# franioli/icepy4d

Hardware: AMD Instinct MI355X
Metric: matched stereo image-pairs/sec (4096 kpts, 1080p) (higher is better)
Workload: dtype f32

## Files before the change

### icepy4d_amd/csrc/attention_bx.hip

```cpp
#include "bf16x3.h"
#include "common.h"
#include "kernels.h"
#include "sp_post.h"

#include <cstdlib>

namespace im {

static constexpr int BKT = 32;
static constexpr int BKS = 144;
static constexpr int BVS = 192;
static constexpr int BK_PLANE = BKT * BKS, BV_PLANE = BKT * BVS;
static constexpr int B_STAGE = 3 * BK_PLANE + 3 * BV_PLANE;
static constexpr int B_LDS = 2 * B_STAGE;
static constexpr int DPL = BKT * 128;
static constexpr int D_LDS = 3 * 3 * (DPL + DPL);

__device__ __forceinline__ f32x16 mfma_attn(u32x4 a, u32x4 b, f32x16 c) {
#ifdef BX_ABL_NO_MFMA
    c[0] += __uint_as_float(a.x ^ b.x);
    return c;
#else
    return mfma_bf(a, b, c);
#endif
}

__device__ __forceinline__ void stage4(unsigned char* plane0, int plane_bytes, int off, float4 x) {
    unsigned h0, m0, l0, h1, m1, l1;
    split2(x.x, x.y, h0, m0, l0);
    split2(x.z, x.w, h1, m1, l1);
    *reinterpret_cast<u32x2*>(plane0 + off) = u32x2{h0, h1};
    *reinterpret_cast<u32x2*>(plane0 + plane_bytes + off) = u32x2{m0, m1};
    *reinterpret_cast<u32x2*>(plane0 + 2 * plane_bytes + off) = u32x2{l0, l1};
}

typedef __attribute__((address_space(3))) bf16x4 lds_bf16x4;
__device__ __forceinline__ u32x2 tr_read(const unsigned char* p) {
#ifdef BX_ABL_NO_VREAD
    const unsigned x = (unsigned)(unsigned long long)p;
    return u32x2{x, 0x3f803f80u};
#else
    const bf16x4 v = __builtin_amdgcn_ds_read_tr16_b64_v4bf16((lds_bf16x4*)(p));
    return __builtin_bit_cast(u32x2, v);
#endif
}
__device__ __forceinline__ u32x4 kf_read(const unsigned char* p) {
#ifdef BX_ABL_NO_KREAD
    const unsigned x = (unsigned)(unsigned long long)p;
    return u32x4{x, 0x3f803f80u, x, 0x3f803f80u};
#else
    return *reinterpret_cast<const u32x4*>(p);
#endif
}

static constexpr float BX_SLACK = 8.f;
__device__ __forceinline__ float bmax3(float a, float b, float c) { return __builtin_fmaxf(__builtin_fmaxf(a, b), c); }

template <bool TAIL>
__device__ __forceinline__ float softmax_ref(f32x16& s, int kb, int nk, int hh, float& m_run, float& l_run, f32x16& o0, f32x16& o1) {
    if (TAIL) {
#pragma unroll
        for (int r = 0; r < 16; ++r)
            if (kb + acc_row(r, hh) >= nk) s[r] = -INFINITY;
    }
    float mx0 = bmax3(s[0], s[1], s[2]), mx1 = bmax3(s[3], s[4], s[5]);
    mx0 = bmax3(mx0, s[6], s[7]); mx1 = bmax3(mx1, s[8], s[9]);
    mx0 = bmax3(mx0, s[10], s[11]); mx1 = bmax3(mx1, s[12], s[13]);
    float mx = bmax3(mx0, mx1, fmaxf(s[14], s[15]));
    mx = fmaxf(mx, __shfl_xor(mx, 32));
    if (__builtin_amdgcn_ballot_w64(mx > m_run + BX_SLACK) != 0) {
        asm volatile("" ::: "memory");
        const float m_new = fmaxf(m_run, mx);
        const float alpha = __builtin_amdgcn_exp2f(m_run - m_new);
        l_run *= alpha;
        o0 *= alpha;
        o1 *= alpha;
        m_run = m_new;
    }
    return (TAIL && m_run == -INFINITY) ? 0.f : m_run;
}
__device__ __forceinline__ void softmax_exp(f32x16& s, float m_use, float& l_run) {
    float r0 = 0.f, r1 = 0.f;
#pragma unroll
    for (int r = 0; r < 16; r += 2) {
        s[r] = __builtin_amdgcn_exp2f(s[r] - m_use);
        s[r + 1] = __builtin_amdgcn_exp2f(s[r + 1] - m_use);
        r0 += s[r]; r1 += s[r + 1];
    }
    float rs = r0 + r1;
    rs += __shfl_xor(rs, 32);
    l_run += rs;
}

__global__ __launch_bounds__(256) void kv_planes_kernel(AttnArgs a) {
    const long rid = (long)blockIdx.x * 32 + (threadIdx.x >> 3);
    const int d8 = threadIdx.x & 7;
    const long per_image = (long)a.heads * a.n_max;
    if (rid >= per_image * a.batch) return;
    const int z = (int)(rid / per_image), rem = (int)(rid - (long)z * per_image), head = rem / a.n_max, row = rem - head * a.n_max;
    if (a.active && a.active[(z >> 1) * a.pstride] == 0) return;
    const int n = a.n_ptr ? a.n_ptr[(z >> 1) * a.pstride + (z & 1)] : a.n_max;
    if (row >= n) return;
    const float* src = (blockIdx.y ? a.v : a.k) + (long)z * a.bstride + (long)head * a.hstride + (long)row * 64 + d8 * 8;
    const float4 u = *reinterpret_cast<const float4*>(src), w = *reinterpret_cast<const float4*>(src + 4);
    const Planes p = split8(u.x, u.y, u.z, u.w, w.x, w.y, w.z, w.w);
    unsigned char* dst = reinterpret_cast<unsigned char*>(a.planes) + ((long)blockIdx.y * per_image * a.batch + rid) * 384 + d8 * 16;
    *reinterpret_cast<u32x4*>(dst) = p.h;
    *reinterpret_cast<u32x4*>(dst + 128) = p.m;
    *reinterpret_cast<u32x4*>(dst + 256) = p.l;
}

template <bool PRE, bool DMA>
__global__ __launch_bounds__(256, 2) void flash_attn_bx_kernel(AttnArgs a) {
    static_assert(PRE || !DMA, "the DMA form stages planes");
    extern __shared__ __attribute__((aligned(16))) unsigned char bsm[];
    constexpr int RD = DMA ? 3 : 2;
    constexpr int KS = DMA ? 128 : BKS, VS = DMA ? 128 : BVS;
    constexpr int KPL = BKT * KS, VPL = BKT * VS;

    const int gsz = (a.batch % 2 == 0) ? 2 : a.batch;
    const int hz = a.heads * gsz;
    const int nqb = (a.n_max + 127) / 128;
    const int per_group = hz * nqb * (a.part ? ATTN_MAX_SPLIT : 1);
    const int grp_idx = blockIdx.x / per_group;
    const int bid = blockIdx.x - grp_idx * per_group;
    const int head = (bid % hz) % a.heads, z = grp_idx * gsz + (bid % hz) / a.heads;
    const int y = a.cross ? (z ^ 1) : z;
    if (a.active && a.active[(z >> 1) * a.pstride] == 0) return;
    const int nq = a.n_ptr ? a.n_ptr[(z >> 1) * a.pstride + (z & 1)] : a.n_max;
    const int nk_all = a.n_ptr ? a.n_ptr[(y >> 1) * a.pstride + (y & 1)] : a.n_max;
    const int qblk = (bid / hz) % nqb, split = (bid / hz) / nqb;
    const int qb = qblk * 128;
    if (qb >= nq || nk_all <= 0) return;
    int n_split = 1, k0 = 0, nk = nk_all;
    if (a.part) {
        const int steps_all = (nk_all + BKT - 1) / BKT;
        const int want = nq > 2048 ? 1 : (nq > 1024 ? 2 : ATTN_MAX_SPLIT);
        const int steps_per = (steps_all + want - 1) / want;
        n_split = (steps_all + steps_per - 1) / steps_per;
        k0 = split * steps_per * BKT;
        nk = min(nk_all - k0, steps_per * BKT);
    }
    if (split >= n_split) return;

    const int tid = threadIdx.x, lane = tid & 63, wave = tid >> 6;
    const int c = lane & 31, hh = lane >> 5;
    const int qrow = qb + wave * 32 + c;

    const float* Q = a.q + (long)z * a.bstride + (long)head * a.hstride;
    __amdgpu_buffer_rsrc_t K, V;
    u32x4 Kd = {}, Vd = {};
    if constexpr (PRE) {
        const long rows = (long)a.heads * a.n_max * a.batch;
        const unsigned char* kp = reinterpret_cast<const unsigned char*>(a.planes) + (((long)y * a.heads + head) * a.n_max + k0) * 384;
        K = make_rsrc(kp, nk * 384);
        V = make_rsrc(kp + rows * 384, nk * 384);
        if constexpr (DMA) { Kd = make_rsrc4(kp, nk * 384); Vd = make_rsrc4(kp + rows * 384, nk * 384); }
    } else {
        K = make_rsrc(a.k + (long)y * a.bstride + (long)head * a.hstride + (long)k0 * 64, nk * 256);
        V = make_rsrc(a.v + (long)y * a.bstride + (long)head * a.hstride + (long)k0 * 64, nk * 256);
    }

    u32x4 qh[4], qm[4], ql[4];
    {
        const float* qp = Q + (long)min(qrow, nq - 1) * 64 + hh * 8;
        const float c2 = a.scale * 1.4426950408889634f;
#pragma unroll
        for (int s = 0; s < 4; ++s) {
            const float4 u = *reinterpret_cast<const float4*>(qp + 16 * s), w = *reinterpret_cast<const float4*>(qp + 16 * s + 4);
            const Planes p = split8(u.x * c2, u.y * c2, u.z * c2, u.w * c2, w.x * c2, w.y * c2, w.z * c2, w.w * c2);
            qh[s] = p.h; qm[s] = p.m; ql[s] = p.l;
        }
    }

    f32x16 o0, o1;
#pragma unroll
    for (int r = 0; r < 16; ++r) { o0[r] = 0.f; o1[r] = 0.f; }
    float m_run = -INFINITY, l_run = 0.f;
    const int nt = (nk + BKT - 1) / BKT;

    unsigned char* const kring = bsm;
    unsigned char* const vring = bsm + RD * 3 * KPL;
    int kq[4], dv[2];
    const int vq = (lane & 15) >> 2;
    if constexpr (DMA) {
#pragma unroll
        for (int s4 = 0; s4 < 4; ++s4) kq[s4] = c * 128 + (((2 * s4 + hh) ^ ((c >> 1) & 7)) << 4);
        const int base = (4 * hh + vq) * 128 + (((lane >> 4) & 1) * 2 + ((lane & 3) >> 1)) * 16 + (lane & 1) * 8, sv = (vq >> 1) & 1;
        dv[0] = base + sv * 64; dv[1] = base + (1 - sv) * 64;
    } else {
#pragma unroll
        for (int s4 = 0; s4 < 4; ++s4) kq[s4] = c * BKS + hh * 16 + 32 * s4;
        const int base = (4 * hh + vq) * BVS + ((lane >> 4) & 1) * 32 + (lane & 3) * 8;
        dv[0] = base; dv[1] = base + 64;
    }

    u32x4 pk[3], pv[3];
    float4 fk[2], fv[2];
    int lk[3], lv[3];
    if constexpr (PRE) {
#pragma unroll
        for (int i = 0; i < 3; ++i) {
            const int id = tid + 256 * i, row = id / 24, rem = id - 24 * row;
            lk[i] = (rem >> 3) * BK_PLANE + row * BKS + (rem & 7) * 16;
            lv[i] = (rem >> 3) * BV_PLANE + row * BVS + (rem & 7) * 16;
        }
    }
    const unsigned voff = PRE ? tid * 16u : ((tid >> 4) * 64 + (tid & 15) * 4) * 4u;
    const int st_k = (tid >> 4) * BKS + (tid & 15) * 8, st_v = (tid >> 4) * BVS + (tid & 15) * 8;
    auto load_k = [&](int tile) {
        if constexpr (PRE) {
            const unsigned so = (unsigned)tile * (BKT * 384u);
#pragma unroll
            for (int i = 0; i < 3; ++i) pk[i] = __builtin_amdgcn_raw_buffer_load_b128(K, voff, so + 4096u * i, 0);
        } else {
            const unsigned so = (unsigned)tile * (BKT * 256u);
// ... 276 lines not shown
            unsigned long long* cp = a.clock + 2 * (blockIdx.x % CLOCK_PROBE_SLOTS);
            cp[0] = ck1 - ck0; cp[1] = cr1 - cr0;
        }
    }
    {
        const int t = nt - 1;
        m_use = softmax_ref<true>(sc, t * BKT, nk, hh, m_run, l_run, o0, o1);
        softmax_exp(sc, m_use, l_run);
        pv_mul(r0, sc);
    }

    if (n_split > 1) {
        const long prow = (((long)z * a.heads + head) * a.n_max + min(qrow, a.n_max - 1)) * 66;
        const long pstride = (long)a.batch * a.heads * a.n_max * 66;
        float* pp = a.part + (long)split * pstride + prow;
        if (qrow < nq) {
#pragma unroll
            for (int g = 0; g < 4; ++g) {
                *reinterpret_cast<float2*>(pp + 8 * g + 4 * hh) = make_float2(o0[4 * g], o0[4 * g + 1]);
                *reinterpret_cast<float2*>(pp + 8 * g + 4 * hh + 2) = make_float2(o0[4 * g + 2], o0[4 * g + 3]);
                *reinterpret_cast<float2*>(pp + 32 + 8 * g + 4 * hh) = make_float2(o1[4 * g], o1[4 * g + 1]);
                *reinterpret_cast<float2*>(pp + 32 + 8 * g + 4 * hh + 2) = make_float2(o1[4 * g + 2], o1[4 * g + 3]);
            }
            if (hh == 0) { pp[64] = m_run; pp[65] = l_run; }
        }
        __threadfence();
        __syncthreads();
        int* flag = reinterpret_cast<int*>(bsm);
        if (tid == 0) {
            int* cnt = a.counters + ((long)z * a.heads + head) * nqb + qblk;
            const int old = atomicAdd(cnt, 1);
            *flag = (old == n_split - 1);
            if (old == n_split - 1) *cnt = 0;
        }
        __syncthreads();
        if (!*flag) return;
        __threadfence();
        float m = -INFINITY;
        for (int sidx = 0; sidx < n_split; ++sidx) m = fmaxf(m, a.part[(long)sidx * pstride + prow + 64]);
        l_run = 0.f;
#pragma unroll
        for (int r = 0; r < 16; ++r) { o0[r] = 0.f; o1[r] = 0.f; }
        for (int sidx = 0; sidx < n_split; ++sidx) {
            const float* ps = a.part + (long)sidx * pstride + prow;
            const float w = __builtin_amdgcn_exp2f(ps[64] - m);
            l_run += w * ps[65];
#pragma unroll
            for (int g = 0; g < 4; ++g)
#pragma unroll
                for (int q = 0; q < 4; ++q) {
                    o0[4 * g + q] += w * ps[8 * g + 4 * hh + q];
                    o1[4 * g + q] += w * ps[32 + 8 * g + 4 * hh + q];
                }
        }
    }

    if (qrow < nq) {
        const float inv = 1.f / l_run;
        float* op = a.out + (long)z * a.out_bstride + (long)qrow * a.ldo + head * 64;
#pragma unroll
        for (int g = 0; g < 4; ++g) {
            const float4 w0 = make_float4(o0[4 * g] * inv, o0[4 * g + 1] * inv, o0[4 * g + 2] * inv, o0[4 * g + 3] * inv);
            const float4 w1 = make_float4(o1[4 * g] * inv, o1[4 * g + 1] * inv, o1[4 * g + 2] * inv, o1[4 * g + 3] * inv);
            *reinterpret_cast<float4*>(op + 8 * g + 4 * hh) = w0;
            *reinterpret_cast<float4*>(op + 32 + 8 * g + 4 * hh) = w1;
        }
    }
}

hipError_t launch_attn_planes(const AttnArgs& a, hipStream_t s) {
    static const bool f32_form = [] { const char* e = getenv("IM_ATTN_F32"); return e && atoi(e) != 0; }();
    if (!a.planes || a.n_max <= 0 || f32_form || a.f32_form) return hipSuccess;
    const long rows = (long)a.batch * a.heads * a.n_max;
    hipLaunchKernelGGL(kv_planes_kernel, dim3((unsigned)((rows + 31) / 32), 2), dim3(256), 0, s, a);
    return hipGetLastError();
}

hipError_t launch_flash_attn_bx(const AttnArgs& a, hipStream_t s) {
    static size_t lds_pre[IM_MAX_DEVICES] = {0}, lds_cut[IM_MAX_DEVICES] = {0};
    dim3 grid(((a.n_max + 127) / 128) * a.heads * a.batch * (a.part ? ATTN_MAX_SPLIT : 1)), block(256);
    static size_t lds_dma[IM_MAX_DEVICES] = {0};
    static const bool reg_staging = [] { const char* e = getenv("IM_ATTN_REG_STAGING"); return e && atoi(e) != 0; }();
    if (a.planes && !reg_staging) {
        if (hipError_t e = ensure_dyn_lds(reinterpret_cast<const void*>(&flash_attn_bx_kernel<true, true>), D_LDS, lds_dma); e != hipSuccess) return e;
        hipLaunchKernelGGL((flash_attn_bx_kernel<true, true>), grid, block, D_LDS, s, a);
    } else if (a.planes) {
        if (hipError_t e = ensure_dyn_lds(reinterpret_cast<const void*>(&flash_attn_bx_kernel<true, false>), B_LDS, lds_pre); e != hipSuccess) return e;
        hipLaunchKernelGGL((flash_attn_bx_kernel<true, false>), grid, block, B_LDS, s, a);
    } else {
        if (hipError_t e = ensure_dyn_lds(reinterpret_cast<const void*>(&flash_attn_bx_kernel<false, false>), B_LDS, lds_cut); e != hipSuccess) return e;
        hipLaunchKernelGGL((flash_attn_bx_kernel<false, false>), grid, block, B_LDS, s, a);
    }
    return hipGetLastError();
}

}
```

### icepy4d_amd/csrc/capi.hip

```cpp
#include "ctx.h"

#include <cstdio>
#include <cstdlib>
#include <cstring>

using namespace im;

extern "C" {

int im_version(void) { return 100; }

int im_ctx_create(int device, im_ctx** out) {
    if (!out) return -1;
    int ndev = 0;
    if (hipGetDeviceCount(&ndev) != hipSuccess || device < 0 || device >= ndev) return -2;
    if (hipSetDevice(device) != hipSuccess) return -3;
    im_ctx* c = new im_ctx();
    c->device = device;
    const char* g = getenv("IM_DEBUG_GUARDS");
    c->guards_on = g && g[0] == '1';
    *out = c;
    return 0;
}

// ... 16 lines not shown
    return 0;
}

int im_ffn_fused(im_ctx* ctx, int act, float* d_x, const float* d_att, const float* h_w0, const float* h_b0, const float* h_ln_g,
                   const float* h_ln_b, const float* h_w3, const float* h_b3, int n_images, int n_rows, const int32_t* d_n, void* stream) {
    IM_CHECK_CTX(ctx);
    if (n_images < 1 || n_rows < 1 || act < 0 || act > 1 || (act == 0 && (!h_ln_g || !h_ln_b))) return ctx->fail(-12, "im_ffn_fused: bad arguments");
    if (act == 1) h_ln_g = h_ln_b = h_b0;
    const std::vector<float> p0 = pack_frag_weights(h_w0, 512, 512), p3 = pack_frag_weights(h_w3, 256, 512);
    const size_t sizes[6] = {p0.size(), 512, 512, 512, p3.size(), 256};
    const float* src[6] = {p0.data(), h_b0, h_ln_g, h_ln_b, p3.data(), h_b3};
    float* d[6] = {nullptr, nullptr, nullptr, nullptr, nullptr, nullptr};
    hipError_t e = hipSuccess;
    for (int i = 0; i < 6 && e == hipSuccess; ++i) {
        e = hipMalloc(&d[i], sizes[i] * sizeof(float));
        if (e == hipSuccess) e = hipMemcpy(d[i], src[i], sizes[i] * sizeof(float), hipMemcpyHostToDevice);
    }
    hipStream_t st = (hipStream_t)stream;
    if (e == hipSuccess) {
        FfnArgs f;
        f.act = act; f.x = d_x; f.x_bstride = (long)n_rows * 256; f.att = d_att; f.att_bstride = (long)n_rows * 256;
        f.w0p = d[0]; f.b0 = d[1]; f.ln_g = d[2]; f.ln_b = d[3]; f.w3p = d[4]; f.b3 = d[5];
        f.m_max = n_rows; f.batch = n_images; f.m_ptr = d_n; f.pstride = 2;
        e = ctx->timed("ffn_fused", st, [&] { return launch_ffn_fused(f, st); });
    }
    const hipError_t e2 = hipStreamSynchronize(st);
    for (int i = 0; i < 6; ++i) hipFree(d[i]);
    IM_HIP(ctx, e);
    IM_HIP(ctx, e2);
    return 0;
}

static int conv3x3_entry(im_ctx* ctx, bool wino, const float* d_in, const float* h_weight, const float* h_bias, float* d_out,
                         int b, int h, int w, int cin, int cout, int relu, int pool, void* stream);

int im_conv3x3(im_ctx* ctx, const float* d_in, const float* h_weight, const float* h_bias, float* d_out, int b, int h,
               int w, int cin, int cout, int relu, int pool, void* stream) {
    return conv3x3_entry(ctx, false, d_in, h_weight, h_bias, d_out, b, h, w, cin, cout, relu, pool, stream);
}

int im_conv3x3_winograd(im_ctx* ctx, const float* d_in, const float* h_weight, const float* h_bias, float* d_out, int b,
                        int h, int w, int cin, int cout, int relu, int pool, void* stream) {
    return conv3x3_entry(ctx, true, d_in, h_weight, h_bias, d_out, b, h, w, cin, cout, relu, pool, stream);
}

static int conv3x3_entry(im_ctx* ctx, bool wino, const float* d_in, const float* h_weight, const float* h_bias, float* d_out,
                         int b, int h, int w, int cin, int cout, int relu, int pool, void* stream) {
    IM_CHECK_CTX(ctx);
    if (cin % 16 || cout % 64) return ctx->fail(-10, "im_conv3x3: cin %% 16 and cout %% 64 must be 0");
    std::vector<float> packed = wino ? pack_conv3x3_wino(h_weight, cout, cin) : pack_conv3x3(h_weight, cout, cin);
    std::vector<float> planes = wino ? pack_conv3x3_wino_bx(h_weight, cout, cin) : std::vector<float>(1);
    const size_t sizes[3] = {packed.size(), (size_t)cout, planes.size()};
    const float* src[3] = {packed.data(), h_bias, planes.data()};
    float* d[3] = {nullptr, nullptr, nullptr};
    hipError_t e = hipSuccess;
    for (int i = 0; i < 3 && e == hipSuccess; ++i) {
        e = hipMalloc(&d[i], sizes[i] * sizeof(float));
        if (e == hipSuccess) e = hipMemcpy(d[i], src[i], sizes[i] * sizeof(float), hipMemcpyHostToDevice);
    }
    hipStream_t st = (hipStream_t)stream;
    if (e == hipSuccess) {
        ConvArgs a;
        a.in = d_in; a.w = d[0]; a.bias = d[1]; a.out = d_out; a.B = b; a.H = h; a.W = w; a.Cin = cin; a.Cout = cout;
        a.relu = relu; a.pool = pool;
        if (wino) a.wx = d[2];
        e = ctx->timed(wino ? "conv_wino" : "conv_direct", st, [&] { return wino ? launch_conv3x3_wino(a, st) : launch_conv3x3(a, st); });
    }
    const hipError_t e2 = hipStreamSynchronize(st);
    for (int i = 0; i < 3; ++i) hipFree(d[i]);
    IM_HIP(ctx, e);
    IM_HIP(ctx, e2);
    return 0;
}

int im_flash_attn(im_ctx* ctx, const float* d_q, const float* d_k, const float* d_v, float* d_out, const int32_t* d_n,
                  int n_max, int batch, int heads, int cross, float scale, void* stream) {
    IM_CHECK_CTX(ctx);
    AttnArgs a;
    a.q = d_q; a.k = d_k; a.v = d_v; a.hstride = (long)n_max * 64; a.bstride = a.hstride * heads;
    a.out = d_out; a.ldo = heads * 64; a.out_bstride = (long)n_max * a.ldo;
    a.n_ptr = d_n; a.n_max = n_max; a.batch = batch; a.heads = heads; a.cross = cross & 1; a.f32_form = (cross >> 1) & 1; a.scale = scale;
    im_ctx::StageScratch& sc = ctx->scratch;
    const bool wants_planes = !(cross & 4) && !a.f32_form;
    IM_GROW(ctx, ctx->grow(sc.attn_part, attn_part_floats(n_max, batch, heads) * sizeof(float), "stage_attn_part"), -11, "im_flash_attn: out of device memory");
    IM_GROW(ctx, ctx->grow(sc.attn_cnt, attn_counter_ints(n_max, batch, heads) * sizeof(int), "stage_attn_cnt", true), -11, "im_flash_attn: out of device memory");
    if (wants_planes) IM_GROW(ctx, ctx->grow(sc.attn_planes, attn_planes_bytes(n_max, batch, heads), "stage_attn_planes"), -11, "im_flash_attn: out of device memory");
    a.part = sc.attn_part.as<float>(); a.counters = sc.attn_cnt.as<int>(); a.planes = wants_planes ? sc.attn_planes.as<unsigned char>() : nullptr;
    IM_HIP(ctx, launch_attn_planes(a, (hipStream_t)stream));
    IM_HIP(ctx, launch_flash_attn(a, (hipStream_t)stream));
    IM_GUARD_CHECK(ctx, (hipStream_t)stream, "im_flash_attn");
    return 0;
}

}
```

### icepy4d_amd/csrc/kernels.h

```cpp
#pragma once
#include <hip/hip_runtime.h>
#include <stdint.h>
#include <vector>

namespace im {

enum GemmEpi {
    EPI_BIAS = 0,
    EPI_BIAS_RESID = 1,
    EPI_HEADS = 2,
    EPI_QKV_ROPE = 3,
    EPI_BIAS_RELU = 4,
    EPI_HEADS_QV = 5,
};

struct GemmArgs {
    const float* A = nullptr;  long a_bstride = 0;  int lda = 0;
    const float* A1 = nullptr; long a1_bstride = 0; int lda1 = 0; int ksplit = 0;
    const float* W = nullptr;  int ldw = 0; long w_bstride = 0;
    const float* bias = nullptr;
    const int* sel = nullptr; long w_sel_stride = 0; long bias_sel_stride = 0;
    int N = 0, K = 0;
    int m_max = 0;
    const int* m_ptr = nullptr;
    const int* n_ptr = nullptr;
    const int* active = nullptr;
    int pstride = 2;
    int pair_batched = 0;
    int batch = 1;
    float alpha = 1.f;
    float* C = nullptr; long c_bstride = 0; int ldc = 0;
    const float* R = nullptr; long r_bstride = 0; int ldr = 0;
    float* q = nullptr; float* k = nullptr; float* v = nullptr; long head_bstride = 0; long head_stride = 0;
    const float* cs = nullptr; const float* sn = nullptr; long enc_bstride = 0;
    int epi = EPI_BIAS;
    int big_tile = 0;
    int bx = 0;
    const void* wp = nullptr;
};
hipError_t launch_gemm(const GemmArgs& a, hipStream_t s);
hipError_t launch_proj_rows(const GemmArgs& a, hipStream_t s);

struct FfnArgs {
    int act = 0;
    float* x = nullptr; long x_bstride = 0;
    const float* att = nullptr; long att_bstride = 0;
    const float* w0p = nullptr; const float* b0 = nullptr;
    const float* ln_g = nullptr; const float* ln_b = nullptr;
    const float* w3p = nullptr; const float* b3 = nullptr;
    int m_max = 0; int batch = 1;
    const int* m_ptr = nullptr;
    const int* active = nullptr;
    int pstride = 2;
};
hipError_t launch_ffn_fused(const FfnArgs& a, hipStream_t s);
std::vector<float> pack_frag_weights(const float* w, int n, int k);

struct AttnArgs {
    const float* q = nullptr; const float* k = nullptr; const float* v = nullptr;
    long bstride = 0; long hstride = 0;
    float* out = nullptr; long out_bstride = 0; int ldo = 256;
    const int* n_ptr = nullptr;
    int pstride = 2;
    int n_max = 0; int batch = 2; int heads = 4; int cross = 0;
    float scale = 1.f;
    const int* active = nullptr;
    float* part = nullptr;
    int* counters = nullptr;
    void* planes = nullptr;
    int f32_form = 0;
    unsigned long long* clock = nullptr;
};
static constexpr int CLOCK_PROBE_SLOTS = 4096;
static constexpr int ATTN_MAX_SPLIT = 4;
inline size_t attn_part_floats(int n_max, int batch, int heads) { return (size_t)ATTN_MAX_SPLIT * batch * heads * n_max * 66; }
inline size_t attn_planes_bytes(int n_max, int batch, int heads) { return (size_t)2 * batch * heads * n_max * 384; }
inline size_t attn_counter_ints(int n_max, int batch, int heads) { return (size_t)batch * heads * ((n_max + 127) / 128); }
hipError_t launch_flash_attn(const AttnArgs& a, hipStream_t s);
hipError_t launch_attn_planes(const AttnArgs& a, hipStream_t s);
hipError_t launch_flash_attn_bx(const AttnArgs& a, hipStream_t s);

struct ConvArgs {
    const float* in = nullptr;
    const float* w = nullptr;
    const float* bias = nullptr;
    float* out = nullptr;
    int B = 1, H = 0, W = 0, Cin = 0, Cout = 0;
    int pool = 0;
    int relu = 1;
    const uint8_t* img = nullptr;
    int img_channels = 1;
    int gray_mode = 0;
    const float* w1 = nullptr;
    const float* b1 = nullptr;
    const float* w1q = nullptr;
    const void* wx = nullptr;
    int f32_form = 0;
    unsigned long long* clock = nullptr;
};
hipError_t launch_conv3x3(const ConvArgs& a, hipStream_t s);
hipError_t launch_conv3x3_wino(const ConvArgs& a, hipStream_t s);
hipError_t launch_conv3x3_wino_bx2(const ConvArgs& a, hipStream_t s);
hipError_t launch_conv1a(const uint8_t* img, int channels, int gray_mode, const float* w, const float* bias, float* out, int B, int H,
                         int W, hipStream_t s);

}
```

Baseline: 172.5.

## Add wide 256-query flash attention kernel for long sequences

Adds a new attention kernel in which each block handles 256 query rows, two 32-row tiles per wave, so every K/V tile staged in LDS feeds twice as many MFMAs. It uses a 3-deep K ring and a 4-deep V ring filled by DMA, with softmax and next-tile QK work interleaved inside the PV MFMA schedule. The existing 128-row kernel now exits early when the wide path covers sequences above 2048 queries, chosen by CU count or an env override. This trades more registers and a single block per CU for fewer redundant K/V loads. It also adds a second launch and clock-probe plumbing.

```diff
diff --git a/icepy4d_amd/csrc/attention_bx.h b/icepy4d_amd/csrc/attention_bx.h
--- /dev/null
+++ b/icepy4d_amd/csrc/attention_bx.h
@@ -0,0 +1,83 @@
+#pragma once
+#include "bf16x3.h"
+#include "common.h"
+
+namespace im {
+
+static constexpr int BKT = 32;
+static constexpr int BKS = 144;
+static constexpr int BVS = 192;
+static constexpr int BK_PLANE = BKT * BKS, BV_PLANE = BKT * BVS;
+static constexpr int B_STAGE = 3 * BK_PLANE + 3 * BV_PLANE;
+static constexpr int B_LDS = 2 * B_STAGE;
+static constexpr int DPL = BKT * 128;
+static constexpr int D_LDS = 3 * 3 * (DPL + DPL);
+
+__device__ __forceinline__ f32x16 mfma_attn(u32x4 a, u32x4 b, f32x16 c) {
+#ifdef BX_ABL_NO_MFMA
+    c[0] += __uint_as_float(a.x ^ b.x);
+    return c;
+#else
+    return mfma_bf(a, b, c);
+#endif
+}
+
+typedef __attribute__((address_space(3))) bf16x4 lds_bf16x4;
+__device__ __forceinline__ u32x2 tr_read(const unsigned char* p) {
+#ifdef BX_ABL_NO_VREAD
+    const unsigned x = (unsigned)(unsigned long long)p;
+    return u32x2{x, 0x3f803f80u};
+#else
+    const bf16x4 v = __builtin_amdgcn_ds_read_tr16_b64_v4bf16((lds_bf16x4*)(p));
+    return __builtin_bit_cast(u32x2, v);
+#endif
+}
+__device__ __forceinline__ u32x4 kf_read(const unsigned char* p) {
+#ifdef BX_ABL_NO_KREAD
+    const unsigned x = (unsigned)(unsigned long long)p;
+    return u32x4{x, 0x3f803f80u, x, 0x3f803f80u};
+#else
+    return *reinterpret_cast<const u32x4*>(p);
+#endif
+}
+
+static constexpr float BX_SLACK = 8.f;
+__device__ __forceinline__ float bmax3(float a, float b, float c) { return __builtin_fmaxf(__builtin_fmaxf(a, b), c); }
+
+template <bool TAIL>
+__device__ __forceinline__ float softmax_ref(f32x16& s, int kb, int nk, int hh, float& m_run, float& l_run, f32x16& o0, f32x16& o1) {
+    if (TAIL) {
+#pragma unroll
+        for (int r = 0; r < 16; ++r)
+            if (kb + acc_row(r, hh) >= nk) s[r] = -INFINITY;
+    }
+    float mx0 = bmax3(s[0], s[1], s[2]), mx1 = bmax3(s[3], s[4], s[5]);
+    mx0 = bmax3(mx0, s[6], s[7]); mx1 = bmax3(mx1, s[8], s[9]);
+    mx0 = bmax3(mx0, s[10], s[11]); mx1 = bmax3(mx1, s[12], s[13]);
+    float mx = bmax3(mx0, mx1, fmaxf(s[14], s[15]));
+    mx = fmaxf(mx, __shfl_xor(mx, 32));
+    if (__builtin_amdgcn_ballot_w64(mx > m_run + BX_SLACK) != 0) {
+        asm volatile("" ::: "memory");
+        const float m_new = fmaxf(m_run, mx);
+        const float alpha = __builtin_amdgcn_exp2f(m_run - m_new);
+        l_run *= alpha;
+        o0 *= alpha;
+        o1 *= alpha;
+        m_run = m_new;
+    }
+    return (TAIL && m_run == -INFINITY) ? 0.f : m_run;
+}
+__device__ __forceinline__ void softmax_exp(f32x16& s, float m_use, float& l_run) {
+    float r0 = 0.f, r1 = 0.f;
+#pragma unroll
+    for (int r = 0; r < 16; r += 2) {
+        s[r] = __builtin_amdgcn_exp2f(s[r] - m_use);
+        s[r + 1] = __builtin_amdgcn_exp2f(s[r + 1] - m_use);
+        r0 += s[r]; r1 += s[r + 1];
+    }
+    float rs = r0 + r1;
+    rs += __shfl_xor(rs, 32);
+    l_run += rs;
+}
+
+}
diff --git a/icepy4d_amd/csrc/attention_bx.hip b/icepy4d_amd/csrc/attention_bx.hip
--- a/icepy4d_amd/csrc/attention_bx.hip
+++ b/icepy4d_amd/csrc/attention_bx.hip
@@ -1,3 +1,4 @@
+#include "attention_bx.h"
 #include "bf16x3.h"
 #include "common.h"
 #include "kernels.h"
@@ -6,24 +7,6 @@
 #include <cstdlib>
 
 namespace im {
-
-static constexpr int BKT = 32;
-static constexpr int BKS = 144;
-static constexpr int BVS = 192;
-static constexpr int BK_PLANE = BKT * BKS, BV_PLANE = BKT * BVS;
-static constexpr int B_STAGE = 3 * BK_PLANE + 3 * BV_PLANE;
-static constexpr int B_LDS = 2 * B_STAGE;
-static constexpr int DPL = BKT * 128;
-static constexpr int D_LDS = 3 * 3 * (DPL + DPL);
-
-__device__ __forceinline__ f32x16 mfma_attn(u32x4 a, u32x4 b, f32x16 c) {
-#ifdef BX_ABL_NO_MFMA
-    c[0] += __uint_as_float(a.x ^ b.x);
-    return c;
-#else
-    return mfma_bf(a, b, c);
-#endif
-}
 
 __device__ __forceinline__ void stage4(unsigned char* plane0, int plane_bytes, int off, float4 x) {
     unsigned h0, m0, l0, h1, m1, l1;
@@ -34,63 +17,6 @@
     *reinterpret_cast<u32x2*>(plane0 + 2 * plane_bytes + off) = u32x2{l0, l1};
 }
 
-typedef __attribute__((address_space(3))) bf16x4 lds_bf16x4;
-__device__ __forceinline__ u32x2 tr_read(const unsigned char* p) {
-#ifdef BX_ABL_NO_VREAD
-    const unsigned x = (unsigned)(unsigned long long)p;
-    return u32x2{x, 0x3f803f80u};
-#else
-    const bf16x4 v = __builtin_amdgcn_ds_read_tr16_b64_v4bf16((lds_bf16x4*)(p));
-    return __builtin_bit_cast(u32x2, v);
-#endif
-}
-__device__ __forceinline__ u32x4 kf_read(const unsigned char* p) {
-#ifdef BX_ABL_NO_KREAD
-    const unsigned x = (unsigned)(unsigned long long)p;
-    return u32x4{x, 0x3f803f80u, x, 0x3f803f80u};
-#else
-    return *reinterpret_cast<const u32x4*>(p);
-#endif
-}
-
-static constexpr float BX_SLACK = 8.f;
-__device__ __forceinline__ float bmax3(float a, float b, float c) { return __builtin_fmaxf(__builtin_fmaxf(a, b), c); }
-
-template <bool TAIL>
-__device__ __forceinline__ float softmax_ref(f32x16& s, int kb, int nk, int hh, float& m_run, float& l_run, f32x16& o0, f32x16& o1) {
-    if (TAIL) {
-#pragma unroll
-        for (int r = 0; r < 16; ++r)
-            if (kb + acc_row(r, hh) >= nk) s[r] = -INFINITY;
-    }
-    float mx0 = bmax3(s[0], s[1], s[2]), mx1 = bmax3(s[3], s[4], s[5]);
-    mx0 = bmax3(mx0, s[6], s[7]); mx1 = bmax3(mx1, s[8], s[9]);
-    mx0 = bmax3(mx0, s[10], s[11]); mx1 = bmax3(mx1, s[12], s[13]);
-    float mx = bmax3(mx0, mx1, fmaxf(s[14], s[15]));
-    mx = fmaxf(mx, __shfl_xor(mx, 32));
-    if (__builtin_amdgcn_ballot_w64(mx > m_run + BX_SLACK) != 0) {
-        asm volatile("" ::: "memory");
-        const float m_new = fmaxf(m_run, mx);
-        const float alpha = __builtin_amdgcn_exp2f(m_run - m_new);
-        l_run *= alpha;
-        o0 *= alpha;
-        o1 *= alpha;
-        m_run = m_new;
-    }
-    return (TAIL && m_run == -INFINITY) ? 0.f : m_run;
-}
-__device__ __forceinline__ void softmax_exp(f32x16& s, float m_use, float& l_run) {
-    float r0 = 0.f, r1 = 0.f;
-#pragma unroll
-    for (int r = 0; r < 16; r += 2) {
-        s[r] = __builtin_amdgcn_exp2f(s[r] - m_use);
-        s[r + 1] = __builtin_amdgcn_exp2f(s[r + 1] - m_use);
-        r0 += s[r]; r1 += s[r + 1];
-    }
-    float rs = r0 + r1;
-    rs += __shfl_xor(rs, 32);
-    l_run += rs;
-}
 
 __global__ __launch_bounds__(256) void kv_planes_kernel(AttnArgs a) {
     const long rid = (long)blockIdx.x * 32 + (threadIdx.x >> 3);
@@ -132,6 +58,7 @@
     const int qblk = (bid / hz) % nqb, split = (bid / hz) / nqb;
     const int qb = qblk * 128;
     if (qb >= nq || nk_all <= 0) return;
+    if (a.wide && nq > ATTN_WIDE_MIN_Q) return;
     int n_split = 1, k0 = 0, nk = nk_all;
     if (a.part) {
         const int steps_all = (nk_all + BKT - 1) / BKT;
@@ -574,8 +501,22 @@
     static size_t lds_dma[IM_MAX_DEVICES] = {0};
     static const bool reg_staging = [] { const char* e = getenv("IM_ATTN_REG_STAGING"); return e && atoi(e) != 0; }();
     if (a.planes && !reg_staging) {
+        const char* const wide_env = getenv("IM_ATTN_WIDE");
+        AttnArgs b = a;
+        b.wide = !a.narrow && a.n_max > ATTN_WIDE_MIN_Q && !(wide_env && wide_env[0] == '0');
+        if (b.wide && !(wide_env && wide_env[0] == '1')) {
+            static int n_cu[IM_MAX_DEVICES] = {0};
+            int dev = 0;
+            if (hipError_t e = hipGetDevice(&dev); e != hipSuccess) return e;
+            if (dev < 0 || dev >= IM_MAX_DEVICES) return hipErrorInvalidDevice;
+            if (!n_cu[dev])
+                if (hipError_t e = hipDeviceGetAttribute(&n_cu[dev], hipDeviceAttributeMultiprocessorCount, dev); e != hipSuccess) return e;
+            b.wide = (long)((a.n_max + 255) / 256) * a.heads * a.batch >= n_cu[dev];
+        }
+        if (b.wide)
+            if (hipError_t e = launch_flash_attn_bx_wide(b, s); e != hipSuccess) return e;
         if (hipError_t e = ensure_dyn_lds(reinterpret_cast<const void*>(&flash_attn_bx_kernel<true, true>), D_LDS, lds_dma); e != hipSuccess) return e;
-        hipLaunchKernelGGL((flash_attn_bx_kernel<true, true>), grid, block, D_LDS, s, a);
+        hipLaunchKernelGGL((flash_attn_bx_kernel<true, true>), grid, block, D_LDS, s, b);
     } else if (a.planes) {
         if (hipError_t e = ensure_dyn_lds(reinterpret_cast<const void*>(&flash_attn_bx_kernel<true, false>), B_LDS, lds_pre); e != hipSuccess) return e;
         hipLaunchKernelGGL((flash_attn_bx_kernel<true, false>), grid, block, B_LDS, s, a);
diff --git a/icepy4d_amd/csrc/attention_bx_wide.hip b/icepy4d_amd/csrc/attention_bx_wide.hip
--- /dev/null
+++ b/icepy4d_amd/csrc/attention_bx_wide.hip
@@ -0,0 +1,404 @@
+#include "attention_bx.h"
+#include "bf16x3.h"
+#include "common.h"
+#include "kernels.h"
+#include "sp_post.h"
+
+#include <cstdlib>
+
+namespace im {
+
+static constexpr int WQ = 256;
+static constexpr int W_KRD = 3, W_VRD = 4;
+static constexpr int W_LDS = (W_KRD + W_VRD) * 3 * DPL;
+
+#define BXW_PIN(x) asm volatile("" : "+v"(x))
+#define BXW_ACC(x) asm volatile("" : "+a"(x))
+
+__device__ __forceinline__ f32x2 both_halves(float x) {
+    const auto r = __builtin_amdgcn_permlane32_swap(__float_as_uint(x), __float_as_uint(x), false, false);
+    return f32x2{__uint_as_float(r[0]), __uint_as_float(r[1])};
+}
+__device__ __forceinline__ void mfma_s_first(f32x16& d, u32x4 k, u32x4 q) {
+#ifdef BX_ABL_NO_MFMA
+    d = mfma_attn(k, q, f32x16{});
+#else
+    asm volatile("v_mfma_f32_32x32x16_bf16 %0, %1, %2, 0" : "=&v"(d) : "v"(k), "a"(q));
+#endif
+}
+__device__ __forceinline__ void mfma_s(f32x16& d, u32x4 k, u32x4 q) {
+#ifdef BX_ABL_NO_MFMA
+    d = mfma_attn(k, q, d);
+#else
+    asm volatile("v_mfma_f32_32x32x16_bf16 %0, %1, %2, %0" : "+v"(d) : "v"(k), "a"(q));
+#endif
+}
+
+__global__ __launch_bounds__(256, 1) void flash_attn_bx_wide_kernel(AttnArgs a) {
+    extern __shared__ __attribute__((aligned(16))) unsigned char wsm[];
+
+    const int gsz = (a.batch % 2 == 0) ? 2 : a.batch;
+    const int hz = a.heads * gsz;
+    const int nqb = (a.n_max + WQ - 1) / WQ;
+    const int per_group = hz * nqb;
+    const int grp_idx = blockIdx.x / per_group;
+    const int bid = blockIdx.x - grp_idx * per_group;
+    const int head = (bid % hz) % a.heads, z = grp_idx * gsz + (bid % hz) / a.heads;
+    const int y = a.cross ? (z ^ 1) : z;
+    if (a.active && a.active[(z >> 1) * a.pstride] == 0) return;
+    const int nq = a.n_ptr ? a.n_ptr[(z >> 1) * a.pstride + (z & 1)] : a.n_max;
+    const int nk = a.n_ptr ? a.n_ptr[(y >> 1) * a.pstride + (y & 1)] : a.n_max;
+    const int qb = (bid / hz) * WQ;
+    if (nq <= ATTN_WIDE_MIN_Q || qb >= nq || nk <= 0) return;
+
+    const int tid = threadIdx.x, lane = tid & 63, wave = tid >> 6;
+    const int c = lane & 31, hh = lane >> 5;
+    const int qrow0 = qb + wave * 64 + c;
+
+    const float* Q = a.q + (long)z * a.bstride + (long)head * a.hstride;
+    const long rows = (long)a.heads * a.n_max * a.batch;
+    const unsigned char* kpl = reinterpret_cast<const unsigned char*>(a.planes) + (((long)y * a.heads + head) * a.n_max) * 384;
+    const u32x4 Kd = make_rsrc4(kpl, nk * 384), Vd = make_rsrc4(kpl + rows * 384, nk * 384);
+
+    u32x4 qh[2][4], qm[2][4], ql[2][4];
+#pragma unroll
+    for (int tl = 0; tl < 2; ++tl) {
+        const float* qp = Q + (long)min(qrow0 + 32 * tl, nq - 1) * 64 + hh * 8;
+        const float c2 = a.scale * 1.4426950408889634f;
+#pragma unroll
+        for (int s = 0; s < 4; ++s) {
+            const float4 u = *reinterpret_cast<const float4*>(qp + 16 * s), w = *reinterpret_cast<const float4*>(qp + 16 * s + 4);
+            const Planes p = split8(u.x * c2, u.y * c2, u.z * c2, u.w * c2, w.x * c2, w.y * c2, w.z * c2, w.w * c2);
+            qh[tl][s] = p.h; qm[tl][s] = p.m; ql[tl][s] = p.l;
+            BXW_ACC(qh[tl][s]); BXW_ACC(qm[tl][s]); BXW_ACC(ql[tl][s]);
+        }
+    }
+
+    f32x16 o0[2], o1[2];
+    float m_run[2] = {-INFINITY, -INFINITY}, l_run[2] = {0.f, 0.f};
+#pragma unroll
+    for (int tl = 0; tl < 2; ++tl) {
+#pragma unroll
+        for (int r = 0; r < 16; ++r) { o0[tl][r] = 0.f; o1[tl][r] = 0.f; }
+    }
+    const int nt = (nk + BKT - 1) / BKT;
+
+    unsigned char* const kring = wsm;
+    unsigned char* const vring = wsm + W_KRD * 3 * DPL;
+    int kq[4], dv[2];
+    const int vq = (lane & 15) >> 2;
+    {
+#pragma unroll
+        for (int s4 = 0; s4 < 4; ++s4) kq[s4] = c * 128 + (((2 * s4 + hh) ^ ((c >> 1) & 7)) << 4);
+        const int base = (4 * hh + vq) * 128 + (((lane >> 4) & 1) * 2 + ((lane & 3) >> 1)) * 16 + (lane & 1) * 8, sv = (vq >> 1) & 1;
+        dv[0] = base + sv * 64; dv[1] = base + (1 - sv) * 64;
+    }
+    const int drow = 8 * wave + (lane >> 3), dpc = lane & 7;
+    const unsigned dvoff_k = drow * 384u + ((dpc ^ ((drow >> 1) & 7)) << 4), dvoff_v = drow * 384u + ((dpc ^ (((drow >> 1) & 1) << 2)) << 4);
+    const unsigned wave_u = __builtin_amdgcn_readfirstlane(tid >> 6);
+    const unsigned lds_k = __builtin_amdgcn_readfirstlane((unsigned)(unsigned long)(lds_ptr_t)kring) + wave_u * 1024u;
+    const unsigned lds_v = __builtin_amdgcn_readfirstlane((unsigned)(unsigned long)(lds_ptr_t)vring) + wave_u * 1024u;
+    auto dma_k1 = [&](int tile, int stage, int i) {
+        dma16(Kd, __builtin_amdgcn_readfirstlane(lds_k + (unsigned)stage * (3u * DPL) + i * DPL), dvoff_k, __builtin_amdgcn_readfirstlane((unsigned)tile * (BKT * 384u) + i * 128u));
+    };
+    auto dma_v1 = [&](int tile, int stage, int i) {
+        dma16(Vd, __builtin_amdgcn_readfirstlane(lds_v + (unsigned)stage * (3u * DPL) + i * DPL), dvoff_v, __builtin_amdgcn_readfirstlane((unsigned)tile * (BKT * 384u) + i * 128u));
+    };
+    auto dma_k = [&](int tile, int stage) {
+#pragma unroll
+        for (int i = 0; i < 3; ++i) dma_k1(tile, stage, i);
+    };
+    auto dma_v = [&](int tile, int stage) {
+#pragma unroll
+        for (int i = 0; i < 3; ++i) dma_v1(tile, stage, i);
+    };
+    auto qk = [&](int stage, f32x16* out) {
+        const unsigned char* const kp = kring + stage * 3 * DPL;
+        f32x16 xa[2], xb[2];
+#pragma unroll
+        for (int tl = 0; tl < 2; ++tl) {
+#pragma unroll
+            for (int r = 0; r < 16; ++r) { xa[tl][r] = 0.f; xb[tl][r] = 0.f; }
+        }
+#pragma unroll
+        for (int s = 0; s < 4; ++s) {
+            const u32x4 kh = kf_read(kp + kq[s]), km = kf_read(kp + DPL + kq[s]), kl = kf_read(kp + 2 * DPL + kq[s]);
+#pragma unroll
+            for (int tl = 0; tl < 2; ++tl) {
+                f32x16& x = (s & 1) ? xb[tl] : xa[tl];
+                x = mfma_attn(kh, ql[tl][s], x);
+                x = mfma_attn(kl, qh[tl][s], x);
+                x = mfma_attn(km, qm[tl][s], x);
+                x = mfma_attn(kh, qm[tl][s], x);
+                x = mfma_attn(km, qh[tl][s], x);
+                x = mfma_attn(kh, qh[tl][s], x);
+            }
+        }
+        out[0] = xa[0] + xb[0];
+        out[1] = xa[1] + xb[1];
+    };
+    auto pv_mul = [&](int stage, const f32x16* p) {
+        const unsigned char* const vp = vring + stage * 3 * DPL;
+#pragma unroll
+        for (int s = 0; s < 2; ++s) {
+            Planes pp[2];
+#pragma unroll
+            for (int tl = 0; tl < 2; ++tl)
+                pp[tl] = split8(p[tl][8 * s + 0], p[tl][8 * s + 1], p[tl][8 * s + 2], p[tl][8 * s + 3], p[tl][8 * s + 4], p[tl][8 * s + 5], p[tl][8 * s + 6], p[tl][8 * s + 7]);
+#pragma unroll
+            for (int dt = 0; dt < 2; ++dt) {
+                const unsigned char* vb = vp + (16 * s) * 128 + dv[dt];
+                const u32x2 h0 = tr_read(vb), h1 = tr_read(vb + 8 * 128);
+                const u32x2 m0 = tr_read(vb + DPL), m1 = tr_read(vb + DPL + 8 * 128);
+                const u32x2 l0 = tr_read(vb + 2 * DPL), l1 = tr_read(vb + 2 * DPL + 8 * 128);
+                const u32x4 vh = {h0.x, h0.y, h1.x, h1.y}, vm = {m0.x, m0.y, m1.x, m1.y}, vl = {l0.x, l0.y, l1.x, l1.y};
+#pragma unroll
+                for (int tl = 0; tl < 2; ++tl) {
+                    f32x16& o = dt ? o1[tl] : o0[tl];
+                    o = mfma_attn(vh, pp[tl].l, o);
+                    o = mfma_attn(vl, pp[tl].h, o);
+                    o = mfma_attn(vm, pp[tl].m, o);
+                    o = mfma_attn(vh, pp[tl].m, o);
+                    o = mfma_attn(vm, pp[tl].h, o);
+                    o = mfma_attn(vh, pp[tl].h, o);
+                }
+            }
+        }
+    };
+
+    f32x16 sc[2], sn[2];
+    dma_k(0, 0); dma_k(1, 1); dma_v(0, 0);
+    asm volatile("s_waitcnt vmcnt(0)" ::: "memory");
+    __syncthreads();
+    dma_k(2, 2); dma_v(1, 1);
+    qk(0, sc);
+    __syncthreads();
+    dma_v(2, 2); dma_k(3, 0);
+
+    static constexpr int PA[6] = {0, 2, 1, 0, 1, 0}, PB[6] = {2, 0, 1, 1, 0, 0};
+    float m_use[2] = {0.f, 0.f};
+    if (nt >= 2) {
+#pragma unroll
+        for (int tl = 0; tl < 2; ++tl) m_use[tl] = softmax_ref<false>(sc[tl], 0, nk, hh, m_run[tl], l_run[tl], o0[tl], o1[tl]);
+    }
+    int r1 = 1, r2 = 2;
+    u32x4 kf[2][3];
+#pragma unroll
+    for (int pl = 0; pl < 3; ++pl) kf[0][pl] = kf_read(kring + 3 * DPL + pl * DPL + kq[0]);
+    unsigned long long ck0 = 0, cr0 = 0;
+    if (a.clock) { ck0 = __builtin_amdgcn_s_memtime(); cr0 = __builtin_amdgcn_s_memrealtime(); }
+    for (int t = 0; t < nt - 2; ++t) {
+        const unsigned char* const kp = kring + r1 * 3 * DPL;
+        const unsigned char* const vp = vring + (t & 3) * 3 * DPL;
+        const unsigned char* const kn = kring + r2 * 3 * DPL;
+        u32x2 vr[2][6];
+#pragma unroll
+        for (int tl = 0; tl < 2; ++tl) {
+#pragma unroll
+            for (int s = 0; s < 4; ++s) { BXW_ACC(qh[tl][s]); BXW_ACC(qm[tl][s]); BXW_ACC(ql[tl][s]); }
+            BXW_ACC(o0[tl]); BXW_ACC(o1[tl]);
+        }
+        __builtin_amdgcn_sched_barrier(0);
+
+        float ra[2][8], rb[2][8], rsum0[2] = {0.f, 0.f}, rsum1[2] = {0.f, 0.f};
+        unsigned ch[2][8], cm[2][8], cl[2][8];
+        auto expo = [&](int tl, int r) {
+#ifdef BX_ABL_NO_EXPCUT
+            return;
+#endif
+            float x = __builtin_amdgcn_exp2f(sc[tl][r] - m_use[tl]);
+            BXW_PIN(x);
+            sc[tl][r] = x;
+            if (r & 1) rsum1[tl] += x; else rsum0[tl] += x;
+        };
+        auto cut_a_pre = [&](int tl, int i) { BXW_PIN(sc[tl][2 * i]); BXW_PIN(sc[tl][2 * i + 1]); };
+        auto cut_a = [&](int tl, int i) {
+#ifdef BX_ABL_NO_EXPCUT
+            ch[tl][i] = __float_as_uint(sc[tl][2 * i]); cm[tl][i] = __float_as_uint(sc[tl][2 * i + 1]); cl[tl][i] = ch[tl][i]; return;
+#endif
+            const float x = sc[tl][2 * i], yv = sc[tl][2 * i + 1];
+            ch[tl][i] = cvt_pk(x, yv);
+            ra[tl][i] = x - __uint_as_float(ch[tl][i] << 16);
+            rb[tl][i] = yv - __uint_as_float(ch[tl][i] & 0xffff0000u);
+            BXW_PIN(ra[tl][i]); BXW_PIN(rb[tl][i]);
+        };
+        auto cut_b_pre = [&](int tl, int i) { BXW_PIN(ra[tl][i]); BXW_PIN(rb[tl][i]); };
+        auto cut_b = [&](int tl, int i) {
+#ifdef BX_ABL_NO_EXPCUT
+            return;
+#endif
+            cm[tl][i] = cvt_pk(ra[tl][i], rb[tl][i]);
+            ra[tl][i] -= __uint_as_float(cm[tl][i] << 16);
+            rb[tl][i] -= __uint_as_float(cm[tl][i] & 0xffff0000u);
+            BXW_PIN(ra[tl][i]); BXW_PIN(rb[tl][i]);
+        };
+        auto cut_l_pre = [&](int tl, int i) { BXW_PIN(ra[tl][i]); };
+        auto cut_l = [&](int tl, int i) {
+#ifdef BX_ABL_NO_EXPCUT
+            return;
+#endif
+            cl[tl][i] = cvt_pk(ra[tl][i], rb[tl][i]);
+            BXW_PIN(cl[tl][i]);
+        };
+
+        f32x16 xa[2], xb[2];
+#pragma unroll
+        for (int s4 = 0; s4 < 4; ++s4) {
+            if (s4 < 3) {
+#pragma unroll
+                for (int pl = 0; pl < 3; ++pl) kf[(s4 + 1) & 1][pl] = kf_read(kp + pl * DPL + kq[s4 + 1]);
+            }
+#pragma unroll
+            for (int j = 0; j < 6; ++j) {
+                const int slot = 6 * s4 + j;
+#pragma unroll
+                for (int tl = 0; tl < 2; ++tl) {
+                    const u32x4 qv = PB[j] == 0 ? qh[tl][s4] : (PB[j] == 1 ? qm[tl][s4] : ql[tl][s4]);
+                    f32x16& x = (j & 1) ? xb[tl] : xa[tl];
+                    if (slot < 2) mfma_s_first(x, kf[s4 & 1][PA[j]], qv);
+                    else mfma_s(x, kf[s4 & 1][PA[j]], qv);
+                    if (slot < 8) expo(tl, slot);
+                    else if (slot < 16) { if (slot & 1) cut_b(tl, (slot - 8) >> 1); else cut_a(tl, (slot - 8) >> 1); }
+                    else { expo(tl, slot - 8); if (slot < 20) cut_l(tl, slot - 16); }
+                    if (tl == 0 && slot >= 18) vr[0][slot - 18] = tr_read(vp + dv[0] + ((slot - 18) >> 1) * DPL + ((slot - 18) & 1) * 8 * 128);
+                    __builtin_amdgcn_sched_barrier(0);
+                }
+            }
+        }
+        asm volatile("s_waitcnt vmcnt(6)" ::: "memory");
+#ifndef BX_ABL_NO_BARRIER
+        __syncthreads();
+#endif
+        __builtin_amdgcn_sched_barrier(0);
+        float mxn[2] = {0.f, 0.f};
+        bool raise[2] = {false, false};
+#pragma unroll
+        for (int g = 0; g < 4; ++g) {
+            const int ks = g >> 1;
+            const u32x4 vf[3] = {u32x4{vr[g & 1][0].x, vr[g & 1][0].y, vr[g & 1][1].x, vr[g & 1][1].y},
+                                 u32x4{vr[g & 1][2].x, vr[g & 1][2].y, vr[g & 1][3].x, vr[g & 1][3].y},
+                                 u32x4{vr[g & 1][4].x, vr[g & 1][4].y, vr[g & 1][5].x, vr[g & 1][5].y}};
+#pragma unroll
+            for (int j = 0; j < 6; ++j) {
+                const int slot = 6 * g + j;
+#pragma unroll
+                for (int tl = 0; tl < 2; ++tl) {
+                    const u32x4 pp[3] = {u32x4{ch[tl][4 * ks], ch[tl][4 * ks + 1], ch[tl][4 * ks + 2], ch[tl][4 * ks + 3]},
+                                         u32x4{cm[tl][4 * ks], cm[tl][4 * ks + 1], cm[tl][4 * ks + 2], cm[tl][4 * ks + 3]},
+                                         u32x4{cl[tl][4 * ks], cl[tl][4 * ks + 1], cl[tl][4 * ks + 2], cl[tl][4 * ks + 3]}};
+                    if (slot < 8) { if (slot & 1) cut_b_pre(tl, 4 + (slot >> 1)); else cut_a_pre(tl, 4 + (slot >> 1)); }
+                    else if (slot < 12) cut_l_pre(tl, 4 + slot - 8);
+                    if (g & 1) o1[tl] = mfma_attn(vf[PA[j]], pp[PB[j]], o1[tl]);
+                    else o0[tl] = mfma_attn(vf[PA[j]], pp[PB[j]], o0[tl]);
+                    if (slot < 8) { if (slot & 1) cut_b(tl, 4 + (slot >> 1)); else cut_a(tl, 4 + (slot >> 1)); }
+                    else if (slot < 12) cut_l(tl, 4 + slot - 8);
+                    if (slot >= 4 && slot < 12) {
+                        float u0 = xa[tl][2 * (slot - 4)] + xb[tl][2 * (slot - 4)];
+                        BXW_PIN(u0);
+                        float u1 = xa[tl][2 * (slot - 4) + 1] + xb[tl][2 * (slot - 4) + 1];
+                        BXW_PIN(u1);
+                        sn[tl][2 * (slot - 4)] = u0; sn[tl][2 * (slot - 4) + 1] = u1;
+                    }
+                    if (slot >= 12 && slot < 20) {
+                        const int i = slot - 12;
+                        float u = i == 0 ? bmax3(sn[tl][0], sn[tl][1], sn[tl][2]) : (i == 7 ? fmaxf(mxn[tl], sn[tl][15]) : bmax3(mxn[tl], sn[tl][2 * i + 1], sn[tl][2 * i + 2]));
+                        BXW_PIN(u);
+                        mxn[tl] = u;
+                    }
+                    if (slot == 12) {
+                        float rs = rsum0[tl] + rsum1[tl];
+                        BXW_PIN(rs);
+                        const f32x2 h = both_halves(rs);
+                        l_run[tl] += h.x + h.y;
+                        BXW_PIN(l_run[tl]);
+                    }
+                    if (slot == 20) {
+                        const f32x2 h = both_halves(mxn[tl]);
+                        mxn[tl] = fmaxf(h.x, h.y);
+                        BXW_PIN(mxn[tl]);
+                        raise[tl] = __builtin_amdgcn_ballot_w64(mxn[tl] > m_run[tl] + BX_SLACK) != 0;
+                    }
+                    if (tl == 0 && g < 3) {
+                        const int gn = g + 1;
+                        vr[gn & 1][j] = tr_read(vp + (16 * (gn >> 1)) * 128 + dv[gn & 1] + (j >> 1) * DPL + (j & 1) * 8 * 128);
+                    }
+                    if (tl == 1 && g == 3 && j < 3) kf[0][j] = kf_read(kn + j * DPL + kq[0]);
+#ifndef BX_ABL_NO_STAGE
+                    if (tl == 0 && slot >= 12 && slot < 15) dma_v1(t + 3, (t + 3) & 3, slot - 12);
+                    if (tl == 0 && slot >= 15 && slot < 18) dma_k1(t + 4, r1, slot - 15);
+#endif
+                    __builtin_amdgcn_sched_barrier(0);
+                }
+            }
+        }
+#pragma unroll
+        for (int tl = 0; tl < 2; ++tl) {
+            if (__builtin_expect(raise[tl], 0)) {
+                asm volatile("" ::: "memory");
+                const float mx = mxn[tl];
+                const float m_new = fmaxf(m_run[tl], mx);
+                const float alpha = __builtin_amdgcn_exp2f(m_run[tl] - m_new);
+                l_run[tl] *= alpha;
+                o0[tl] *= alpha;
+                o1[tl] *= alpha;
+                m_run[tl] = m_new;
+            }
+            m_use[tl] = m_run[tl];
+            sc[tl] = sn[tl];
+        }
+        r1 = r2; r2 = r2 == 2 ? 0 : r2 + 1;
+    }
+    asm volatile("s_waitcnt vmcnt(0)" ::: "memory");
+    if (nt >= 2) {
+        __syncthreads();
+        qk((nt - 1) % 3, sn);
+#pragma unroll
+        for (int tl = 0; tl < 2; ++tl) softmax_exp(sc[tl], m_use[tl], l_run[tl]);
+        pv_mul((nt - 2) & 3, sc);
+        sc[0] = sn[0]; sc[1] = sn[1];
+    }
+    if (a.clock && nt > 8) {
+        const unsigned long long ck1 = __builtin_amdgcn_s_memtime(), cr1 = __builtin_amdgcn_s_memrealtime();
+        if (threadIdx.x == 0) {
+            unsigned long long* cp = a.clock + 2 * (blockIdx.x % CLOCK_PROBE_SLOTS);
+            cp[0] = ck1 - ck0; cp[1] = cr1 - cr0;
+        }
+    }
+    {
+        const int t = nt - 1;
+#pragma unroll
+        for (int tl = 0; tl < 2; ++tl) {
+            m_use[tl] = softmax_ref<true>(sc[tl], t * BKT, nk, hh, m_run[tl], l_run[tl], o0[tl], o1[tl]);
+            softmax_exp(sc[tl], m_use[tl], l_run[tl]);
+        }
+        pv_mul((nt - 1) & 3, sc);
+    }
+
+#pragma unroll
+    for (int tl = 0; tl < 2; ++tl) {
+        const int qrow = qrow0 + 32 * tl;
+        if (qrow < nq) {
+            const float inv = 1.f / l_run[tl];
+            float* op = a.out + (long)z * a.out_bstride + (long)qrow * a.ldo + head * 64;
+#pragma unroll
+            for (int g = 0; g < 4; ++g) {
+                const float4 w0 = make_float4(o0[tl][4 * g] * inv, o0[tl][4 * g + 1] * inv, o0[tl][4 * g + 2] * inv, o0[tl][4 * g + 3] * inv);
+                const float4 w1 = make_float4(o1[tl][4 * g] * inv, o1[tl][4 * g + 1] * inv, o1[tl][4 * g + 2] * inv, o1[tl][4 * g + 3] * inv);
+                *reinterpret_cast<float4*>(op + 8 * g + 4 * hh) = w0;
+                *reinterpret_cast<float4*>(op + 32 + 8 * g + 4 * hh) = w1;
+            }
+        }
+    }
+}
+#undef BXW_PIN
+#undef BXW_ACC
+
+hipError_t launch_flash_attn_bx_wide(const AttnArgs& a, hipStream_t s) {
+    static size_t lds_wide[IM_MAX_DEVICES] = {0};
+    if (hipError_t e = ensure_dyn_lds(reinterpret_cast<const void*>(&flash_attn_bx_wide_kernel), W_LDS, lds_wide); e != hipSuccess) return e;
+    dim3 grid(((a.n_max + WQ - 1) / WQ) * a.heads * a.batch), block(256);
+    hipLaunchKernelGGL(flash_attn_bx_wide_kernel, grid, block, W_LDS, s, a);
+    return hipGetLastError();
+}
+
+}
diff --git a/icepy4d_amd/csrc/capi.hip b/icepy4d_amd/csrc/capi.hip
--- a/icepy4d_amd/csrc/capi.hip
+++ b/icepy4d_amd/csrc/capi.hip
@@ -122,10 +122,12 @@
     a.n_ptr = d_n; a.n_max = n_max; a.batch = batch; a.heads = heads; a.cross = cross & 1; a.f32_form = (cross >> 1) & 1; a.scale = scale;
     im_ctx::StageScratch& sc = ctx->scratch;
     const bool wants_planes = !(cross & 4) && !a.f32_form;
+    a.narrow = (cross >> 3) & 1;
     IM_GROW(ctx, ctx->grow(sc.attn_part, attn_part_floats(n_max, batch, heads) * sizeof(float), "stage_attn_part"), -11, "im_flash_attn: out of device memory");
     IM_GROW(ctx, ctx->grow(sc.attn_cnt, attn_counter_ints(n_max, batch, heads) * sizeof(int), "stage_attn_cnt", true), -11, "im_flash_attn: out of device memory");
     if (wants_planes) IM_GROW(ctx, ctx->grow(sc.attn_planes, attn_planes_bytes(n_max, batch, heads), "stage_attn_planes"), -11, "im_flash_attn: out of device memory");
     a.part = sc.attn_part.as<float>(); a.counters = sc.attn_cnt.as<int>(); a.planes = wants_planes ? sc.attn_planes.as<unsigned char>() : nullptr;
+    a.clock = ctx->clock_of(0);
     IM_HIP(ctx, launch_attn_planes(a, (hipStream_t)stream));
     IM_HIP(ctx, launch_flash_attn(a, (hipStream_t)stream));
     IM_GUARD_CHECK(ctx, (hipStream_t)stream, "im_flash_attn");
diff --git a/icepy4d_amd/csrc/kernels.h b/icepy4d_amd/csrc/kernels.h
--- a/icepy4d_amd/csrc/kernels.h
+++ b/icepy4d_amd/csrc/kernels.h
@@ -70,15 +70,19 @@
     void* planes = nullptr;
     int f32_form = 0;
     unsigned long long* clock = nullptr;
+    int narrow = 0;
+    int wide = 0;
 };
 static constexpr int CLOCK_PROBE_SLOTS = 4096;
 static constexpr int ATTN_MAX_SPLIT = 4;
+static constexpr int ATTN_WIDE_MIN_Q = 2048;
 inline size_t attn_part_floats(int n_max, int batch, int heads) { return (size_t)ATTN_MAX_SPLIT * batch * heads * n_max * 66; }
 inline size_t attn_planes_bytes(int n_max, int batch, int heads) { return (size_t)2 * batch * heads * n_max * 384; }
 inline size_t attn_counter_ints(int n_max, int batch, int heads) { return (size_t)batch * heads * ((n_max + 127) / 128); }
 hipError_t launch_flash_attn(const AttnArgs& a, hipStream_t s);
 hipError_t launch_attn_planes(const AttnArgs& a, hipStream_t s);
 hipError_t launch_flash_attn_bx(const AttnArgs& a, hipStream_t s);
+hipError_t launch_flash_attn_bx_wide(const AttnArgs& a, hipStream_t s);
 
 struct ConvArgs {
     const float* in = nullptr;
```

Result: no change. 172.4 (-0.0%).
